# lmcinnes/pynndescent

Measured on AMD Instinct MI355X. Metric: index build: points indexed/sec (recall@10 vs brute force reported alongside), higher is better.
Workload: dtype f32

## Files before the change

include/pynnd_amd.h:

```cpp
#ifndef PYNND_AMD_H
#define PYNND_AMD_H

#include <stdint.h>

#ifdef __cplusplus
extern "C" {
#endif

#define NND_METRIC_SQEUCLIDEAN 0
#define NND_METRIC_ALT_COSINE 1
#define NND_METRIC_ALT_DOT 2
#define NND_METRIC_ALT_INNER_PRODUCT 3
#define NND_METRIC_CORRELATION 4
#define NND_METRIC_ALT_HELLINGER 5
enum { NND_METRIC_PROXY_INNER_PRODUCT = 6 };

#define NND_ABI_VERSION 6

typedef struct nnd_handle_s *nnd_handle_t;

typedef struct nnd_params {
    int64_t n;
    int32_t dim;
    int32_t metric;
    int32_t n_neighbors;
    int32_t n_trees;
    int32_t leaf_size;
    int32_t max_depth;
    int32_t max_candidates;
    int32_t n_iters;
    float delta;
    int64_t rng_state[3];
    int64_t tree_rng[3];
    int32_t device;
    int32_t join_blocks;
    int32_t flags;
    int32_t reserved[5];
} nnd_params;

#define NND_FLAG_NO_GRAPH 1
#define NND_FLAG_NO_PREP 2
#define NND_FLAG_TEST_SELECT_WAVE 4
#define NND_FLAG_TEST_SMALL_REGIONS 8
#define NND_FLAG_TEST_ROUTE_PLAIN 16
#define NND_FLAG_TEST_FOREST_BY_TREE 32
#define NND_FLAG_TEST_FAIL 64
#define NND_FLAG_TEST_VANISH 128
#define NND_FLAG_TEST_SAMPLE_ATOMIC 256
#define NND_FLAG_TEST_FOREST_FALLBACK_TOPS 512
#define NND_FLAG_TEST_FOREST_FALLBACK_SHARE 1024
#define NND_TEST_FALLBACK_AT(flags) ((((flags) & 512) ? 1 : 0) + (((flags) & 1024) ? 2 : 0))
#define NND_FLAG_TEST_SAMPLE_NOMEM 2048
#define NND_FLAG_TEST_SELECT_HALF 4096
#define NND_FLAG_TEST_GATHER_INLINE 8192
#define NND_FLAG_TEST_JOIN_UNSTAGED 16384

#define NND_FLAG_TEST_EXACT_F64 32768

typedef struct nnd_stats {
    int64_t n_iters_run;
    int64_t n_leaves;
    int64_t tree_levels;
    int64_t leaf_pairs;
    int64_t leaf_rows;
    int64_t join_pairs[64];
    int64_t join_rows[64];
    int64_t join_active[64];
    int64_t proposals[64];
    int64_t updates[64];
    float ms_prep, ms_forest, ms_leaf_init, ms_random_init, ms_descent, ms_finalize;
    float ms_sample[64], ms_join[64], ms_merge[64];
    int64_t join_mfma[64];
    int64_t leaf_mfma;
    int64_t n_cells;
    int64_t join_substeps[64];
} nnd_stats;

int32_t nnd_abi_version(void);
const char *nnd_last_global_error(void);
const char *nnd_last_error(nnd_handle_t h);

int32_t nnd_create(nnd_handle_t *out, const nnd_params *params);
int32_t nnd_destroy(nnd_handle_t h);
int32_t nnd_release_pending(void);

int32_t nnd_host_copy(void *dst, const void *src, int64_t bytes);
int32_t nnd_host_sqrt_f32(float *dst, const float *src, int64_t count);
void *nnd_host_alloc(int64_t bytes);
int32_t nnd_host_free(void *p);

int32_t nnd_set_data_host(nnd_handle_t h, const float *x);
int32_t nnd_set_data_device(nnd_handle_t h, const float *x_dev);
#define NND_DTYPE_FLOAT32 0
#define NND_DTYPE_FLOAT16 1
#define NND_DTYPE_BFLOAT16 2
#define NND_DTYPE_FLOAT64 3
int32_t nnd_set_data_device_typed(nnd_handle_t h, const void *x_dev, int32_t dtype);
int32_t nnd_device_rows_f32(int32_t device, void *hip_stream, const void *src_dev, int32_t dtype, int64_t n, int32_t dim,
                            int32_t normalize, float *dst_dev);
#define NND_CORRECT_COPY 0
#define NND_CORRECT_SQRT 1
#define NND_CORRECT_ALT_COSINE 2
#define NND_CORRECT_ALT_INNER_PRODUCT 3
#define NND_CORRECT_ALT_HELLINGER 4
int32_t nnd_device_correct(int32_t device, void *hip_stream, int32_t kind, const float *in_dev, void *out_dev, int64_t count);
int32_t nnd_device_update_rows(int32_t device, void *hip_stream, int32_t dim, const void *old_dev, int32_t old_dtype, int64_t n_old,
                               const void *fresh_dev, int32_t fresh_dtype, int64_t n_fresh, const void *upd_dev, int32_t upd_dtype,
                               int64_t n_upd, const int32_t *upd_rows_dev, const int32_t *upd_ids_dev, int64_t n_pairs, void *out_dev,
                               int32_t out_dtype);
int32_t nnd_device_update_graph(int32_t device, void *hip_stream, const int32_t *idx_dev, const float *dist_dev, int64_t n_old, int32_t k,
                                const int32_t *upd_ids_dev, int64_t n_upd, int64_t n_new, uint8_t *map_dev, int32_t *out_idx_dev,
                                float *out_dist_dev);
int32_t nnd_device_recall_hits(int32_t device, void *hip_stream, const int32_t *true_idx_dev, int64_t m, int32_t k, const int32_t *graph_idx_dev,
                               int64_t n, int32_t width, const int32_t *rows_dev, int64_t *hits_dev);
int32_t nnd_data_nonfinite(nnd_handle_t h, int32_t *out);
int32_t nnd_data_negative(nnd_handle_t h, int32_t *out);

int32_t nnd_make_forest(nnd_handle_t h);
int32_t nnd_leaf_array_shape(nnd_handle_t h, int64_t *n_leaves, int32_t *max_leaf_size);
int32_t nnd_get_leaf_array(nnd_handle_t h, int32_t *out_host);

int32_t nnd_reset_graph(nnd_handle_t h);
int32_t nnd_init_from_leaves(nnd_handle_t h);
int32_t nnd_init_from_leaf_array(nnd_handle_t h, const int32_t *leaf_array, int64_t n_leaves, int32_t max_leaf_size);
int32_t nnd_init_random(nnd_handle_t h);
int32_t nnd_init_from_graph(nnd_handle_t h, const int32_t *init_idx, const float *init_dist, int32_t width);
int32_t nnd_init_from_neighbor_graph(nnd_handle_t h, const int32_t *init_idx, const float *init_dist, int32_t width);
int32_t nnd_init_from_graph_device(nnd_handle_t h, const int32_t *init_idx_dev, const float *init_dist_dev, int32_t width);
int32_t nnd_init_from_neighbor_graph_device(nnd_handle_t h, const int32_t *init_idx_dev, const float *init_dist_dev, int32_t width);

int32_t nnd_descent_iter(nnd_handle_t h, int64_t *c_out);
int32_t nnd_descent(nnd_handle_t h);

int32_t nnd_finalize_host(nnd_handle_t h, int32_t *out_idx, float *out_dist);
int32_t nnd_finalize_device(nnd_handle_t h, int32_t *out_idx_dev, float *out_dist_dev);

int32_t nnd_build_device(nnd_handle_t h, int32_t *out_idx_dev, float *out_dist_dev);

int32_t nnd_build(const nnd_params *params, const float *x, const int32_t *init_idx, const float *init_dist,
                  int32_t init_width, int32_t *out_idx, float *out_dist, nnd_stats *stats, char *err,
// ... 167 lines not shown
```

pynndescent_amd/_capi.py:

```python
import ctypes as C
import os

import numpy as np

_HERE = os.path.dirname(os.path.abspath(__file__))
LIB_PATH = os.environ.get("PYNND_AMD_LIB", os.path.join(_HERE, "libpynnd_amd.so"))

NND_METRIC_SQEUCLIDEAN = 0
NND_METRIC_ALT_COSINE = 1
NND_METRIC_ALT_DOT = 2
NND_METRIC_ALT_INNER_PRODUCT = 3
NND_METRIC_CORRELATION = 4
NND_METRIC_ALT_HELLINGER = 5
NND_METRIC_PROXY_INNER_PRODUCT = 6
METRIC_CODES = {"euclidean": NND_METRIC_SQEUCLIDEAN, "l2": NND_METRIC_SQEUCLIDEAN, "sqeuclidean": NND_METRIC_SQEUCLIDEAN,
                "cosine": NND_METRIC_ALT_COSINE, "dot": NND_METRIC_ALT_DOT, "inner_product": NND_METRIC_ALT_INNER_PRODUCT,
                "correlation": NND_METRIC_CORRELATION, "hellinger": NND_METRIC_ALT_HELLINGER,
                "proxy_inner_product": NND_METRIC_PROXY_INNER_PRODUCT}
NND_DTYPE_FLOAT32, NND_DTYPE_FLOAT16, NND_DTYPE_BFLOAT16, NND_DTYPE_FLOAT64 = 0, 1, 2, 3
NND_CORRECT_COPY, NND_CORRECT_SQRT, NND_CORRECT_ALT_COSINE, NND_CORRECT_ALT_INNER_PRODUCT, NND_CORRECT_ALT_HELLINGER = 0, 1, 2, 3, 4
NND_FLAG_NO_GRAPH = 1
NND_FLAG_NO_PREP = 2
NND_FLAG_TEST_SELECT_WAVE = 4
NND_FLAG_TEST_SMALL_REGIONS = 8
NND_FLAG_TEST_ROUTE_PLAIN = 16
NND_FLAG_TEST_FOREST_BY_TREE = 32
NND_FLAG_TEST_FAIL = 64
NND_FLAG_TEST_VANISH = 128
NND_FLAG_TEST_FOREST_FALLBACK_TOPS = 512
NND_FLAG_TEST_FOREST_FALLBACK_SHARE = 1024
NND_FLAG_TEST_GATHER_INLINE = 8192
NND_FLAG_TEST_JOIN_UNSTAGED = 16384
NND_FLAG_TEST_SELECT_HALF = 4096
NND_FLAG_TEST_SAMPLE_NOMEM = 2048
NND_FLAG_TEST_EXACT_F64 = 32768
NND_FLAG_TEST_SAMPLE_ATOMIC = 256


class NNDParams(C.Structure):
    _fields_ = [
        ("n", C.c_int64),
        ("dim", C.c_int32),
        ("metric", C.c_int32),
        ("n_neighbors", C.c_int32),
        ("n_trees", C.c_int32),
        ("leaf_size", C.c_int32),
        ("max_depth", C.c_int32),
        ("max_candidates", C.c_int32),
        ("n_iters", C.c_int32),
        ("delta", C.c_float),
        ("rng_state", C.c_int64 * 3),
        ("tree_rng", C.c_int64 * 3),
        ("device", C.c_int32),
        ("join_blocks", C.c_int32),
        ("flags", C.c_int32),
        ("reserved", C.c_int32 * 5),
    ]


class NNDSearchGraphStats(C.Structure):
    _fields_ = [("forward_nnz", C.c_int64), ("reverse_nnz", C.c_int64), ("union_nnz", C.c_int64), ("final_nnz", C.c_int64),
                ("min_distance", C.c_float), ("max_degree_out", C.c_int32), ("ms_device", C.c_float), ("reserved", C.c_int32 * 3)]


class NNDStats(C.Structure):
    _fields_ = [
        ("n_iters_run", C.c_int64),
        ("n_leaves", C.c_int64),
        ("tree_levels", C.c_int64),
        ("leaf_pairs", C.c_int64),
        ("leaf_rows", C.c_int64),
        ("join_pairs", C.c_int64 * 64),
        ("join_rows", C.c_int64 * 64),
        ("join_active", C.c_int64 * 64),
        ("proposals", C.c_int64 * 64),
        ("updates", C.c_int64 * 64),
        ("ms_prep", C.c_float),
        ("ms_forest", C.c_float),
        ("ms_leaf_init", C.c_float),
        ("ms_random_init", C.c_float),
        ("ms_descent", C.c_float),
        ("ms_finalize", C.c_float),
        ("ms_sample", C.c_float * 64),
        ("ms_join", C.c_float * 64),
        ("ms_merge", C.c_float * 64),
        ("join_mfma", C.c_int64 * 64),
        ("leaf_mfma", C.c_int64),
        ("n_cells", C.c_int64),
        ("join_substeps", C.c_int64 * 64),
    ]

    def as_dict(self):
        it = int(self.n_iters_run)
        m = min(it, 64)
        out = {
            "n_iters_run": it, "n_leaves": int(self.n_leaves), "tree_levels": int(self.tree_levels),
            "leaf_pairs": int(self.leaf_pairs), "leaf_rows": int(self.leaf_rows), "leaf_mfma": int(self.leaf_mfma), "n_cells": int(self.n_cells),
        }
        for name in ("join_pairs", "join_rows", "join_active", "proposals", "updates", "join_mfma", "join_substeps"):
            out[name] = [int(v) for v in getattr(self, name)[:m]]
        for name in ("ms_prep", "ms_forest", "ms_leaf_init", "ms_random_init", "ms_descent", "ms_finalize"):
            out[name] = float(getattr(self, name))
        for name in ("ms_sample", "ms_join", "ms_merge"):
            out[name] = [float(v) for v in getattr(self, name)[:m]]
        return out


class NNDShardInfo(C.Structure):
    _fields_ = [
        ("n_total", C.c_int64), ("own_lo", C.c_int64), ("own_hi", C.c_int64),
        ("world", C.c_int32), ("rank", C.c_int32), ("local_trees", C.c_int32), ("iters", C.c_int32),
        ("c", C.c_int64 * 64),
        ("offer_records", C.c_int64 * 64),
        ("proposal_records", C.c_int64 * 64),
        ("deferred", C.c_int64 * 64),
        ("dropped_offers", C.c_int64),
        ("bytes_sent", C.c_int64),
        ("ms_total", C.c_float), ("ms_allgather", C.c_float), ("ms_klist_exchange", C.c_float),
# ... 780 lines not shown
```

pynndescent_amd/csrc/finalize.hip:

```cpp
#include "common.h"
#include "metric.h"
#include "state.h"

template <int FAM>
__device__ __forceinline__ void fin_acc(int metric, double a, double b, double &dot, double &nx, double &ny) {
    nnd_ref_acc<FAM, NND_HELLINGER_F32>(metric, a, b, dot, nx, ny);
}
template <int FAM>
__device__ __forceinline__ float fin_value(int metric, double dot, double nx, double ny) {
    const double dt = nnd_group_sum_f64<16>(dot);
    if (metric == 0) return (float)dt;
    return (float)nnd_ref_dist<FAM>(metric, dt, nnd_group_sum_f64<16>(nx), nnd_group_sum_f64<16>(ny));
}

template <int METRIC>
__global__ __launch_bounds__(256, METRIC == 0 ? 6 : 4) void k_finalize(const float *__restrict__ x, int d, int64_t lo, int64_t n, int k, int ks,
                                                  const uint32_t *__restrict__ knn_e, const int32_t *__restrict__ order,
                                                  int32_t *__restrict__ out_idx, float *__restrict__ out_dist) {
    const int lane = nnd_lane(), w = threadIdx.x >> 6;
    int64_t b = blockIdx.x;
    if ((gridDim.x & 7) == 0) b = (b & 7) * (gridDim.x >> 3) + (b >> 3);
    const int64_t g = lo + b * 4 + w;
    if (g >= n) return;
    const int64_t v = order ? (int64_t)order[g] : g;
    uint32_t e = lane < k ? knn_e[v * ks + lane] : NND_EMPTY_E;
    const float *xv = x + v * d;
    const int grp = lane >> 4, l16 = lane & 15;
    const bool vec = (d & 3) == 0;
    constexpr int metric = METRIC, FAM = METRIC < 2 ? NND_CODES_01 : NND_CODES_ANY;
    float mine = INFINITY;
    const int nsteps = (k + 3) >> 2;
    for (int s0 = 0; s0 < nsteps; s0 += 4) {
        const float *xu[4];
        bool on[4];
        double dot[4], nx[4], ny[4];
#pragma unroll
        for (int u = 0; u < 4; u++) {
            const int j = 4 * (s0 + u) + grp;
            const uint32_t ej = __shfl(e, j & 63, 64);
            on[u] = j < k && ej != NND_EMPTY_E;
            xu[u] = x + (int64_t)(on[u] ? (ej & NND_IDX_MASK) : 0) * d;
            dot[u] = nx[u] = ny[u] = 0.0;
        }
        double mua = 0.0, mub[4] = {0.0, 0.0, 0.0, 0.0};
        if (metric == 4) {
            mua = nnd_row_mean_f64<16>(xv, d, l16);
#pragma unroll
            for (int u = 0; u < 4; u++) mub[u] = nnd_row_mean_f64<16>(xu[u], d, l16);
        }
        if (vec) {
            for (int t = 4 * l16; t < d; t += 64) {
                const float4 a = *(const float4 *)(xv + t);
                float4 q[4];
#pragma unroll
                for (int u = 0; u < 4; u++) q[u] = *(const float4 *)(xu[u] + t);
#pragma unroll
                for (int u = 0; u < 4; u++) {
                    const double a0 = a.x, a1 = a.y, a2 = a.z, a3 = a.w;
                    const double b0 = q[u].x, b1 = q[u].y, b2 = q[u].z, b3 = q[u].w;
                    if (metric == 0) {
                        dot[u] += (a0 - b0) * (a0 - b0) + (a1 - b1) * (a1 - b1) + (a2 - b2) * (a2 - b2) + (a3 - b3) * (a3 - b3);
                    } else if (metric == 1) {
                        dot[u] += a0 * b0 + a1 * b1 + a2 * b2 + a3 * b3;
                        nx[u] += a0 * a0 + a1 * a1 + a2 * a2 + a3 * a3;
                        ny[u] += b0 * b0 + b1 * b1 + b2 * b2 + b3 * b3;
                    } else {
                        fin_acc<FAM>(metric, a0 - mua, b0 - mub[u], dot[u], nx[u], ny[u]);
                        fin_acc<FAM>(metric, a1 - mua, b1 - mub[u], dot[u], nx[u], ny[u]);
                        fin_acc<FAM>(metric, a2 - mua, b2 - mub[u], dot[u], nx[u], ny[u]);
                        fin_acc<FAM>(metric, a3 - mua, b3 - mub[u], dot[u], nx[u], ny[u]);
                    }
                }
            }
        } else {
            for (int t = l16; t < d; t += 16) {
                const double a0 = xv[t];
#pragma unroll
                for (int u = 0; u < 4; u++) {
                    fin_acc<FAM>(metric, a0 - mua, (double)xu[u][t] - mub[u], dot[u], nx[u], ny[u]);
                }
            }
        }
#pragma unroll
        for (int u = 0; u < 4; u++) {
            float val = fin_value<FAM>(metric, dot[u], nx[u], ny[u]);
            if (!on[u]) val = INFINITY;
            const float got = __shfl(val, 16 * (lane & 3), 64);
            if ((lane >> 2) == s0 + u) mine = got;
        }
    }
    const uint32_t myidx = e == NND_EMPTY_E ? NND_IDX_MASK : (e & NND_IDX_MASK);
    const uint64_t mykey = ((uint64_t)__float_as_uint(mine) << 32) | myidx;
    int r = 0;
    for (int j = 0; j < k; j++) {
        uint64_t kj = ((uint64_t)__float_as_uint(__shfl(mine, j, 64)) << 32) | __shfl(myidx, j, 64);
        r += (kj < mykey || (kj == mykey && j < lane)) ? 1 : 0;
    }
    if (lane < k) {
        out_idx[(v - lo) * k + r] = e == NND_EMPTY_E ? -1 : (int32_t)(e & NND_IDX_MASK);
        out_dist[(v - lo) * k + r] = mine;
    }
}

template <bool XM>
__global__ __launch_bounds__(256) void k_finalize_wide(const float *__restrict__ x, int d, int64_t lo, int64_t n, int k, int ks, int metric,
                                                       const uint32_t *__restrict__ knn_e, int32_t *__restrict__ out_idx,
                                                       float *__restrict__ out_dist) {
    __shared__ uint32_t sid[4][NND_WIDE_K];
    __shared__ float sdist[4][NND_WIDE_K];
    constexpr int FAM = XM ? NND_CODES_ANY : NND_CODES_01;
    const int lane = nnd_lane(), w = threadIdx.x >> 6, grp = lane >> 4, l16 = lane & 15;
    const int64_t v = lo + (int64_t)blockIdx.x * 4 + w;
    if (v >= n) return;
    for (int j = lane; j < k; j += 64) sid[w][j] = knn_e[v * ks + j];
    nnd_wave_lds_sync();
    const float *xv = x + v * d;
    for (int j0 = 0; j0 < k; j0 += 4) {
        const int j = j0 + grp;
        const uint32_t ej = j < k ? sid[w][j] : NND_EMPTY_E;
        const bool on = ej != NND_EMPTY_E;
        const float *xu = x + (int64_t)(on ? (ej & NND_IDX_MASK) : 0) * d;
        double dot = 0.0, nx = 0.0, ny = 0.0;
        const bool corr = XM && metric == 4;
        const double mua = corr ? nnd_row_mean_f64<16>(xv, d, l16) : 0.0, mub = corr ? nnd_row_mean_f64<16>(xu, d, l16) : 0.0;
        for (int t = l16; t < d; t += 16) fin_acc<FAM>(metric, (double)xv[t] - mua, (double)xu[t] - mub, dot, nx, ny);
        float val = fin_value<FAM>(metric, dot, nx, ny);
        if (!on) val = INFINITY;
        if (l16 == 0 && j < k) sdist[w][j] = val;
    }
    nnd_wave_lds_sync();
    for (int j = lane; j < k; j += 64) {
        const uint32_t e = sid[w][j];
        const uint32_t myidx = e == NND_EMPTY_E ? NND_IDX_MASK : (e & NND_IDX_MASK);
        const uint64_t mykey = ((uint64_t)__float_as_uint(sdist[w][j]) << 32) | myidx;
        int r = 0;
        for (int q = 0; q < k; q++) {
            const uint32_t eq = sid[w][q];
            const uint64_t kq = ((uint64_t)__float_as_uint(sdist[w][q]) << 32) | (eq == NND_EMPTY_E ? NND_IDX_MASK : (eq & NND_IDX_MASK));
            r += (kq < mykey || (kq == mykey && q < j)) ? 1 : 0;
        }
        out_idx[(v - lo) * k + r] = e == NND_EMPTY_E ? -1 : (int32_t)(e & NND_IDX_MASK);
        out_dist[(v - lo) * k + r] = sdist[w][j];
    }
}

int nnd_launch_finalize(nnd_ctx *ctx, int32_t *out_idx_dev, float *out_dist_dev) {
    unsigned grid = (unsigned)((ctx->own_hi - ctx->own_lo + 3) / 4);
    if (ctx->k > 64) {
        hipLaunchKernelGGL(ctx->p.metric >= 2 ? k_finalize_wide<true> : k_finalize_wide<false>, dim3(grid), dim3(256), 0, ctx->stream, ctx->x_orig, ctx->d, ctx->own_lo, ctx->own_hi, ctx->k, ctx->ks,
                           ctx->p.metric, ctx->knn_e, out_idx_dev, out_dist_dev);
        NND_HIP_CHECK(hipGetLastError());
        return 0;
    }
    grid = (grid + 7u) & ~7u;
    auto kern = k_finalize<0>;
    switch (ctx->p.metric) {
        case 1: kern = k_finalize<1>; break;
        case 2: kern = k_finalize<2>; break;
        case 3: kern = k_finalize<3>; break;
        case 4: kern = k_finalize<4>; break;
        case 5: kern = k_finalize<5>; break;
        case 6: kern = k_finalize<6>; break;
    }
    hipLaunchKernelGGL(kern, dim3(grid), dim3(256), 0, ctx->stream, ctx->x_orig, ctx->d, ctx->own_lo, ctx->own_hi,
                       ctx->k, ctx->ks, ctx->knn_e, nnd_vertex_order(ctx), out_idx_dev, out_dist_dev);
    NND_HIP_CHECK(hipGetLastError());
    return 0;
}

__global__ __launch_bounds__(64) void k_pairwise(const float *__restrict__ xp, int dp, const float *__restrict__ nrm,
                                                 int metric, const int32_t *__restrict__ rows_a, int na,
                                                 const int32_t *__restrict__ rows_b, int nb, float *__restrict__ out) {
    const int lane = nnd_lane(), r16 = lane & 15, g = lane >> 4;
    const int ta = blockIdx.y, tb = blockIdx.x;
    int ia = ta * 16 + r16, ib = tb * 16 + r16;
    int ida = ia < na ? rows_a[ia] : -1, idb = ib < nb ? rows_b[ib] : -1;
    f32x4 acc = {0.f, 0.f, 0.f, 0.f};
    for (int t = 0; t < (dp >> 4); t++) {
        int c = 4 * t + g;
        float4 a = ida >= 0 ? *(const float4 *)(xp + (int64_t)ida * dp + 4 * c) : make_float4(0, 0, 0, 0);
        float4 b = idb >= 0 ? *(const float4 *)(xp + (int64_t)idb * dp + 4 * c) : make_float4(0, 0, 0, 0);
        acc = __builtin_amdgcn_mfma_f32_16x16x4f32(a.x, b.x, acc, 0, 0, 0);
        acc = __builtin_amdgcn_mfma_f32_16x16x4f32(a.y, b.y, acc, 0, 0, 0);
        acc = __builtin_amdgcn_mfma_f32_16x16x4f32(a.z, b.z, acc, 0, 0, 0);
        acc = __builtin_amdgcn_mfma_f32_16x16x4f32(a.w, b.w, acc, 0, 0, 0);
    }
    int col = tb * 16 + r16;
    float nbv = idb >= 0 ? nrm[idb] : 0.0f;
#pragma unroll
    for (int r = 0; r < 4; r++) {
        int row = ta * 16 + 4 * g + r;
        int idr = row < na ? rows_a[row] : -1;
        if (row < na && col < nb) out[(int64_t)row * nb + col] = nnd_gram_to_dist<NND_CODES_ANY>(metric, acc[r], idr >= 0 ? nrm[idr] : 0.0f, nbv);
    }
}

int nnd_launch_pairwise(nnd_ctx *ctx, const int32_t *rows_a_dev, int na, const int32_t *rows_b_dev, int nb, float *out_dev) {
    dim3 grid((nb + 15) / 16, (na + 15) / 16);
    hipLaunchKernelGGL(k_pairwise, grid, dim3(64), 0, ctx->stream, ctx->xp, ctx->dp, ctx->nrm, ctx->p.metric, rows_a_dev, na,
                       rows_b_dev, nb, out_dev);
    NND_HIP_CHECK(hipGetLastError());
    return 0;
}
```

pynndescent_amd/csrc/merge.hip:

```cpp
#include "common.h"
#include "metric.h"
#include "merge.h"
#include "state.h"

__global__ __launch_bounds__(256) void k_merge(uint64_t *__restrict__ pbuf, uint8_t *__restrict__ pdirty, int pcap,
                                               int64_t lo, int64_t n, int k, int ks, uint32_t *__restrict__ knn_e,
                                               float *__restrict__ knn_d, float *__restrict__ th,
                                               long long *__restrict__ counters) {
    __shared__ int wacc[4];
    const int lane = nnd_lane(), w = threadIdx.x >> 6;
    const int64_t base = lo + ((int64_t)blockIdx.x * 4 + w) * 64;
    int acc = 0;
    unsigned long long m = 0;
    if (base < n) m = __ballot(base + lane < n && pdirty[base + lane < n ? base + lane : lo] != 0);
    struct pair_t {
        int64_t v[2];
        uint64_t key[2];
        uint32_t e[2];
        float d[2];
    };
    auto fetch = [&](pair_t &p) __attribute__((always_inline)) {
#pragma unroll
        for (int u = 0; u < 2; u++) {
            p.v[u] = -1;
// ... 74 lines not shown
    quad_t cur, nxt;
    cur.v = nxt.v = -1;
    bool have = m != 0;
    if (have) fetch(cur);
    while (have) {
        have = m != 0;
        if (have) fetch(nxt);
        const bool on = cur.v >= 0;
        const int64_t v = on ? cur.v : lo;
        const uint32_t e0 = on ? cur.e : NND_EMPTY_E;
        const float d0 = on ? cur.d : INFINITY;
        acc += nnd_merge_rows_q16<NB>(on, knn_e + v * ks, knn_d + v * ks, th + v, e0, d0, k, PCAP,
                                      [&](int c, uint32_t &id, float &dc) {
                                          const int b = c >> 4;
                                          const uint64_t kk = b == 0 ? cur.key[0] : (b == 1 ? cur.key[1] : (b == 2 ? cur.key[2] : cur.key[3]));
                                          id = nnd_key_idx(kk);
                                          dc = nnd_key_dist(kk);
                                          return kk != NND_EMPTY_KEY;
                                      });
        if (on) {
#pragma unroll
            for (int b = 0; b < NB; b++)
                if (cur.key[b] != NND_EMPTY_KEY) pbuf[v * PCAP + b * 16 + j] = NND_EMPTY_KEY;
            if (j == 0) pdirty[v] = 0;
        }
        cur = nxt;
    }
    if (lane == 0) wacc[w] = acc;
    __syncthreads();
    if (threadIdx.x == 0) {
        const long long a = (long long)wacc[0] + wacc[1] + wacc[2] + wacc[3];
        if (a) nnd_count(counters, CNT_ACCEPT, a);
    }
}

__global__ __launch_bounds__(256) void k_merge_wide(uint64_t *__restrict__ pbuf, uint8_t *__restrict__ pdirty, int pcap, int64_t lo, int64_t n,
                                                    int k, int ks, uint32_t *__restrict__ knn_e, float *__restrict__ knn_d,
                                                    float *__restrict__ th, long long *__restrict__ counters) {
    __shared__ uint64_t scr[4][NND_WIDE_SCRATCH_WORDS];
    __shared__ int wacc[4];
    const int lane = nnd_lane(), w = threadIdx.x >> 6;
    const int64_t base = lo + ((int64_t)blockIdx.x * 4 + w) * 64;
    int acc = 0;
    unsigned long long m = 0;
    if (base < n) m = __ballot(base + lane < n && pdirty[base + lane < n ? base + lane : lo] != 0);
    while (m) {
        const int64_t v = base + __builtin_ctzll(m);
        m &= m - 1;
        const uint64_t mykey = lane < pcap ? pbuf[v * pcap + lane] : NND_EMPTY_KEY;
        acc += nnd_merge_row_lds<1>(scr[w], knn_e + v * ks, knn_d + v * ks, th + v, k, pcap, [&](int c, uint32_t &id, float &dc) {
            id = nnd_key_idx(mykey);
            dc = nnd_key_dist(mykey);
            return mykey != NND_EMPTY_KEY;
        });
        if (lane < pcap && mykey != NND_EMPTY_KEY) pbuf[v * pcap + lane] = NND_EMPTY_KEY;
        if (lane == 0) pdirty[v] = 0;
        nnd_wave_lds_sync();
    }
    if (lane == 0) wacc[w] = acc;
    __syncthreads();
    if (threadIdx.x == 0) {
        const long long a = (long long)wacc[0] + wacc[1] + wacc[2] + wacc[3];
        if (a) nnd_count(counters, CNT_ACCEPT, a);
    }
}

int nnd_launch_merge(nnd_ctx *ctx) {
    if (ctx->pcap > 64) { ctx->set_error("k_merge expects at most 64 proposal slots per row"); return 1; }
    const dim3 grid((unsigned)((ctx->own_hi - ctx->own_lo + 255) / 256));
    if (ctx->k > NND_MAX_K)
        hipLaunchKernelGGL(k_merge_wide, grid, dim3(256), 0, ctx->stream, ctx->pbuf, ctx->pdirty, ctx->pcap, ctx->own_lo, ctx->own_hi, ctx->k,
                           ctx->ks, ctx->knn_e, ctx->knn_d, ctx->th, ctx->counters);
    else if (ctx->k <= 16 && ctx->pcap == 64)
        hipLaunchKernelGGL(k_merge_q, grid, dim3(256), 0, ctx->stream, ctx->pbuf, ctx->pdirty, ctx->own_lo, ctx->own_hi, ctx->k, ctx->ks,
                           ctx->knn_e, ctx->knn_d, ctx->th, ctx->counters);
    else
    hipLaunchKernelGGL(k_merge, grid, dim3(256), 0, ctx->stream, ctx->pbuf,
                       ctx->pdirty, ctx->pcap, ctx->own_lo, ctx->own_hi, ctx->k, ctx->ks, ctx->knn_e, ctx->knn_d, ctx->th, ctx->counters);
    NND_HIP_CHECK(hipGetLastError());
    if (ctx->n_ranks <= 1) ctx->pbuf_clean = true;
    return 0;
}

__global__ __launch_bounds__(256) void k_random_init(const float *__restrict__ xp, int dp, const float *__restrict__ nrm,
                                                     int metric, int64_t n, int64_t lo, int64_t hi, int k, int ks,
                                                     const uint32_t *__restrict__ knn_e, uint32_t seed,
                                                     uint64_t *__restrict__ pbuf, uint8_t *__restrict__ pdirty, int pcap) {
    const int lane = nnd_lane(), w = threadIdx.x >> 6;
    const int64_t v = lo + (int64_t)blockIdx.x * 4 + w;
    if (v >= hi) return;
    int filled = 0;
    for (int j0 = 0; j0 < k; j0 += 64) {
        const uint32_t e = j0 + lane < k ? knn_e[v * ks + j0 + lane] : NND_EMPTY_E;
        filled += __popcll(__ballot(e != NND_EMPTY_E));
    }
    int todo = k - filled;
    if (todo <= 0) return;
    if (todo > 64) todo = 64;
    uint32_t pick = (uint32_t)(nnd_hash3(seed, (uint32_t)v, (uint32_t)lane) % (uint64_t)n);
    bool mine = lane < todo;
    for (int j = 0; j < todo; j++) {
        uint32_t other = __shfl(pick, j, 64);
        if (j < lane && other == pick) mine = false;
    }
    for (int j = 0; j < todo; j++) {
        uint32_t id = __shfl(pick, j, 64);
        bool on = __shfl((int)mine, j, 64);
        if (!on) continue;
        float d = nnd_row_pair_dist(xp, dp, nrm, metric, v, (int64_t)id);
        if (lane == 0) pbuf[v * pcap + j] = nnd_make_key(d, id);
    }
    if (lane == 0) pdirty[v] = 1;
}

int nnd_launch_random_init(nnd_ctx *ctx) {
    for (int pass = 0; pass < (ctx->k + 63) / 64; pass++) {
        ctx->pbuf_clean = false;
        hipLaunchKernelGGL(k_random_init, dim3((unsigned)((ctx->own_hi - ctx->own_lo + 3) / 4)), dim3(256), 0, ctx->stream, ctx->xp,
                           ctx->dp, ctx->nrm, ctx->p.metric, ctx->n, ctx->own_lo, ctx->own_hi, ctx->k, ctx->ks, ctx->knn_e,
                           ctx->seed ^ 0x3C6EF372u ^ (uint32_t)(pass * 0x9E3779B9u), ctx->pbuf, ctx->pdirty, ctx->pcap);
        NND_HIP_CHECK(hipGetLastError());
        if (nnd_launch_merge(ctx)) return 1;
    }
    return 0;
}

__global__ __launch_bounds__(256) void k_graph_init(const float *__restrict__ xp, int dp, const float *__restrict__ nrm,
                                                    int metric, int64_t n, int64_t lo, int64_t hi, const int32_t *__restrict__ gidx,
                                                    const float *__restrict__ gdist, int width, int col0, int wchunk,
                                                    uint64_t *__restrict__ pbuf, uint8_t *__restrict__ pdirty, int pcap) {
    const int lane = nnd_lane(), w = threadIdx.x >> 6;
    const int64_t v = lo + (int64_t)blockIdx.x * 4 + w;
    if (v >= hi) return;
    gidx += -lo * width;
    if (gdist) gdist += -lo * width;
    int32_t id = lane < wchunk ? gidx[v * width + col0 + lane] : -1;
    bool mine = id >= 0 && (int64_t)id < n;
    for (int j = 0; j < wchunk; j++) {
        int32_t other = __shfl(id, j, 64);
        if (j < lane && other == id) mine = false;
    }
    for (int j = 0; j < wchunk; j++) {
        int32_t q = __shfl(id, j, 64);
        bool on = __shfl((int)mine, j, 64);
        if (!on) continue;
        float d = gdist ? nnd_clamp_dist(gdist[v * width + col0 + j]) : nnd_row_pair_dist(xp, dp, nrm, metric, v, (int64_t)q);
        if (lane == 0) pbuf[v * pcap + j] = nnd_make_key(d, (uint32_t)q);
    }
    if (lane == 0) pdirty[v] = 1;
}

int nnd_launch_init_from_graph(nnd_ctx *ctx, const int32_t *idx_dev, const float *dist_dev, int width) {
    if (ctx->pcap < 64) { ctx->set_error("init graphs need 64 proposal slots per row"); return 1; }
    const int64_t rows = ctx->own_hi - ctx->own_lo;
    if (rows <= 0) return 0;
    for (int col0 = 0; col0 < width; col0 += 64) {
        const int wchunk = width - col0 < 64 ? width - col0 : 64;
        ctx->pbuf_clean = false;
        hipLaunchKernelGGL(k_graph_init, dim3((unsigned)((rows + 3) / 4)), dim3(256), 0, ctx->stream, ctx->xp, ctx->dp,
                           ctx->nrm, ctx->p.metric, ctx->n, ctx->own_lo, ctx->own_hi, idx_dev, dist_dev, width, col0, wchunk, ctx->pbuf, ctx->pdirty,
                           ctx->pcap);
        NND_HIP_CHECK(hipGetLastError());
        if (nnd_launch_merge(ctx)) return 1;
    }
    return 0;
}

__global__ void k_clear_new_flags(uint32_t *__restrict__ knn_e, int64_t lo, int64_t hi, int ks) {
    int64_t t = lo * ks + (int64_t)blockIdx.x * blockDim.x + threadIdx.x;
    if (t >= hi * ks) return;
    const uint32_t e = knn_e[t];
    if (e != NND_EMPTY_E) knn_e[t] = e & NND_IDX_MASK;
}
int nnd_launch_clear_new_flags(nnd_ctx *ctx) {
    const int64_t total = (ctx->own_hi - ctx->own_lo) * ctx->ks;
    if (total <= 0) return 0;
    hipLaunchKernelGGL(k_clear_new_flags, dim3((unsigned)((total + 255) / 256)), dim3(256), 0, ctx->stream, ctx->knn_e,
                       ctx->own_lo, ctx->own_hi, ctx->ks);
    NND_HIP_CHECK(hipGetLastError());
    return 0;
}


__global__ void k_import_proposals(const uint64_t *__restrict__ keys, const int32_t *__restrict__ targets, int64_t count,
                                   uint64_t *__restrict__ pbuf, uint8_t *__restrict__ pdirty, int pcap, uint32_t slot_seed,
                                   const uint32_t *__restrict__ knn_e, const float *__restrict__ th, int ks) {
    const int64_t i = (int64_t)blockIdx.x * blockDim.x + threadIdx.x;
    if (i >= count) return;
    const uint64_t key = keys[i];
    const int64_t t = targets[i];
    if (t < 0) return;
    const uint32_t src = nnd_key_idx(key);
    if (!(nnd_key_dist(key) < th[t])) return;
    const u32x4 *row = (const u32x4 *)(knn_e + t * ks);
    bool present = false;
    for (int c = 0; c < (ks >> 2); c++) {
        const u32x4 wv = row[c] & NND_IDX_MASK;
        present |= (wv.x == src) | (wv.y == src) | (wv.z == src) | (wv.w == src);
    }
    if (present) return;
    const uint32_t s = nnd_hash2(slot_seed, src) & (uint32_t)(pcap - 1);
    atomicMin((unsigned long long *)&pbuf[t * pcap + s], (unsigned long long)key);
    pdirty[t] = 1;
// ... 260 lines not shown
```

pynndescent_amd/csrc/prep.hip:

```cpp
#include "common.h"
#include "metric.h"
#include "state.h"

#define NND_MEAN_ROWS 65536
__global__ void k_colsum_partial(const float *__restrict__ x, int64_t row0, int64_t r_lo, int64_t r_hi, int64_t stride, int d,
                                 int rows_per_block, double *__restrict__ partial) {
    __shared__ float wmax[4];
    int64_t r0 = r_lo + (int64_t)blockIdx.x * rows_per_block;
    int64_t r1 = r0 + rows_per_block < r_hi ? r0 + rows_per_block : r_hi;
    float mx = 0.0f;
    for (int j = threadIdx.x; j < d; j += blockDim.x) {
        double s = 0.0;
        for (int64_t r = r0; r < r1; r++) {
            const float v = x[(r * stride - row0) * d + j];
            s += (double)v;
            mx = fmaxf(mx, fabsf(v));
        }
        partial[(int64_t)blockIdx.x * (d + 1) + j] = s;
    }
#pragma unroll
    for (int o = 32; o > 0; o >>= 1) mx = fmaxf(mx, __shfl_xor(mx, o, 64));
    if (nnd_lane() == 0) wmax[threadIdx.x >> 6] = mx;
    __syncthreads();
    if (threadIdx.x == 0) {
// ... 200 lines not shown
        hipLaunchKernelGGL(k_colsum_final, dim3(dp + 1), dim3(256), 0, ctx->stream, partial, nblocks, d, dp, n_s, ctx->mean);
    } else {
        NND_HIP_CHECK(hipMemsetAsync(ctx->mean, 0, sizeof(float) * (dp + 4), ctx->stream));
    }
    hipLaunchKernelGGL(k_screen_scale, dim3(1), dim3(64), 0, ctx->stream, ctx->mean, d, dp, ctx->p.metric);
    NND_HIP_CHECK(hipGetLastError());
    return 0;
}
int nnd_prep_partial_blocks(int64_t members) { return (int)((members + 127) / 128); }
double *nnd_prep_partial_buffer(nnd_ctx *ctx, size_t doubles) {
    if (!ctx->mem.grow(&ctx->colsum_partial, &ctx->colsum_cap, doubles, doubles)) ctx->set_error("allocation of the column-sum scratch failed");
    return ctx->colsum_partial;
}
int nnd_prep_rows(nnd_ctx *ctx, const float *x_all, int64_t row_lo, int64_t row_hi, bool first) {
    const int d = ctx->d, dp = ctx->dp;
    const int64_t rows = row_hi - row_lo;
    long long *flag = ctx->counters_sum + CNT_PREP_FLAG;
    if (first) NND_HIP_CHECK(hipMemsetAsync(flag, 0, sizeof(long long), ctx->stream));
    if (rows <= 0) return 0;
    if ((d & 3) == 0 && ((uintptr_t)x_all & 15) == 0) {
        int lpr = 1;
        while (lpr < (dp >> 2) && lpr < 64) lpr <<= 1;
        const int64_t rows_per_wg = 4 * (64 / lpr);
        hipLaunchKernelGGL(k_prep_rows_v4, dim3((unsigned)((rows + rows_per_wg - 1) / rows_per_wg)), dim3(256), 0, ctx->stream, x_all, row_lo, row_hi, d,
                           dp, ctx->p.metric, lpr, ctx->mean, ctx->xp, ctx->nrm, ctx->xh, ctx->nr2, flag);
    } else {
        hipLaunchKernelGGL(k_prep_rows, dim3((unsigned)((rows + 3) / 4)), dim3(256), 0, ctx->stream, x_all, row_lo, row_hi, d, dp,
                           ctx->p.metric, ctx->mean, ctx->xp, ctx->nrm, ctx->xh, ctx->nr2, flag);
    }
    NND_HIP_CHECK(hipGetLastError());
    return 0;
}

int nnd_launch_prep(nnd_ctx *ctx) {
    const int64_t n = ctx->n;
    int64_t n_s, stride;
    nnd_prep_mean_geometry(n, &n_s, &stride);
    int nblocks = 0;
    double *partial = nullptr;
    if (nnd_prep_column_pass(ctx->p.metric)) {
        partial = nnd_prep_partial_buffer(ctx, (size_t)nnd_prep_partial_blocks(n_s) * (ctx->d + 1));
        if (!partial) return 1;
        nblocks = nnd_prep_mean_partial(ctx, ctx->x_orig, 0, 0, n_s, stride, partial);
    }
    if (nnd_prep_mean_finish(ctx, partial, nblocks, n_s)) return 1;
    if (nnd_prep_rows(ctx, ctx->x_orig, 0, n, true)) return 1;
    long long *flag = ctx->counters_sum + CNT_PREP_FLAG;
    NND_HIP_CHECK(hipMemcpyAsync(&ctx->h_pin->data_flags, flag, sizeof(long long), hipMemcpyDeviceToHost, ctx->stream));
    return 0;
}

__global__ void k_reset_graph(uint32_t *__restrict__ e, float *__restrict__ dd, int64_t total, float *__restrict__ th,
                              int64_t n) {
    int64_t i = (int64_t)blockIdx.x * blockDim.x + threadIdx.x;
    if (i < total) {
        e[i] = NND_EMPTY_E;
        dd[i] = INFINITY;
    }
    if (i < n) th[i] = INFINITY;
}

int nnd_launch_reset_graph(nnd_ctx *ctx) {
    ctx->all_new = true;
    ctx->last_updates = -1;
    int64_t total = ctx->n * ctx->ks;
    hipLaunchKernelGGL(k_reset_graph, dim3((unsigned)((total + 255) / 256)), dim3(256), 0, ctx->stream, ctx->knn_e,
                       ctx->knn_d, total, ctx->th, ctx->n);
    if (!ctx->pbuf_clean) {
        NND_HIP_CHECK(hipMemsetAsync(ctx->pbuf + (size_t)ctx->slim_row0() * ctx->pcap, 0xFF, sizeof(uint64_t) * (size_t)ctx->slim_rows() * ctx->pcap, ctx->stream));
        if (ctx->pbuf_r) NND_HIP_CHECK(hipMemsetAsync(ctx->pbuf_r, 0xFF, sizeof(uint64_t) * (size_t)ctx->n * ctx->pcap_r, ctx->stream));
    }
    if (!ctx->rbuf_clean)
        NND_HIP_CHECK(hipMemsetAsync(ctx->rbuf + (size_t)ctx->slim_row0() * 2 * ctx->rcap, 0xFF, sizeof(uint32_t) * (size_t)ctx->slim_rows() * 2 * ctx->rcap, ctx->stream));
    ctx->pbuf_clean = ctx->rbuf_clean = true;
    NND_HIP_CHECK(hipGetLastError());
    ctx->iter = 0;
    return 0;
}

int nnd_zero_counters(nnd_ctx *ctx) {
    NND_HIP_CHECK(hipMemsetAsync(ctx->counters, 0, sizeof(long long) * CNT_COUNT * NND_CNT_STRIPES, ctx->stream));
    return 0;
}
__global__ __launch_bounds__(256) void k_counters_reduce(const long long *__restrict__ counters, long long *__restrict__ out) {
    __shared__ long long red[256];
    for (int c = 0; c < CNT_COUNT; c++) {
        long long s = 0;
        for (int i = threadIdx.x; i < NND_CNT_STRIPES; i += 256) s += counters[(size_t)i * CNT_COUNT + c];
        red[threadIdx.x] = s;
        __syncthreads();
        for (int o = 128; o > 0; o >>= 1) {
            if (threadIdx.x < o) red[threadIdx.x] += red[threadIdx.x + o];
            __syncthreads();
        }
        if (threadIdx.x == 0) out[c] = red[0];
        __syncthreads();
    }
}
int nnd_read_counters(nnd_ctx *ctx) {
    hipLaunchKernelGGL(k_counters_reduce, dim3(1), dim3(256), 0, ctx->stream, ctx->counters, ctx->counters_sum);
    NND_HIP_CHECK(hipGetLastError());
    NND_HIP_CHECK(hipMemcpyAsync(ctx->h_pin->counters, ctx->counters_sum, sizeof(long long) * CNT_COUNT, hipMemcpyDeviceToHost, ctx->stream));
    NND_HIP_CHECK(nnd_sync_spin(ctx));
    for (int c = 0; c < CNT_COUNT; c++) ctx->h_counters[c] = ctx->h_pin->counters[c];
    return 0;
}
```

Baseline: 51.91 million.

## Add 16-lane finalize kernel, ballot-skip full rows in random init, wave-reduce counters

```diff
diff --git a/include/pynnd_amd.h b/include/pynnd_amd.h
--- a/include/pynnd_amd.h
+++ b/include/pynnd_amd.h
@@ -56,6 +56,7 @@
 #define NND_FLAG_TEST_JOIN_UNSTAGED 16384
 
 #define NND_FLAG_TEST_EXACT_F64 32768
+#define NND_FLAG_TEST_RANDOM_INIT_ROWWISE 65536
 
 typedef struct nnd_stats {
     int64_t n_iters_run;
diff --git a/pynndescent_amd/_capi.py b/pynndescent_amd/_capi.py
--- a/pynndescent_amd/_capi.py
+++ b/pynndescent_amd/_capi.py
@@ -34,6 +34,7 @@
 NND_FLAG_TEST_SELECT_HALF = 4096
 NND_FLAG_TEST_SAMPLE_NOMEM = 2048
 NND_FLAG_TEST_EXACT_F64 = 32768
+NND_FLAG_TEST_RANDOM_INIT_ROWWISE = 65536
 NND_FLAG_TEST_SAMPLE_ATOMIC = 256
 
 
diff --git a/pynndescent_amd/csrc/finalize.hip b/pynndescent_amd/csrc/finalize.hip
--- a/pynndescent_amd/csrc/finalize.hip
+++ b/pynndescent_amd/csrc/finalize.hip
@@ -1,6 +1,31 @@
 #include "common.h"
+#include "merge.h"
 #include "metric.h"
 #include "state.h"
+
+__device__ __forceinline__ double fin_sub(double a, double b) {
+#pragma clang fp contract(off)
+    return a - b;
+}
+__device__ __forceinline__ double fin_add(double a, double b) {
+#pragma clang fp contract(off)
+    return a + b;
+}
+__device__ __forceinline__ double fin_chunk(double a0, double a1, double a2, double a3, double b0, double b1, double b2, double b3) {
+#pragma clang fp contract(off)
+    double s = a1 * b1;
+    s = __builtin_fma(a0, b0, s);
+    s = __builtin_fma(a2, b2, s);
+    return __builtin_fma(a3, b3, s);
+}
+__device__ __forceinline__ double fin_chunk_sq(const float4 a, const float4 b) {
+    const double d0 = fin_sub((double)a.x, (double)b.x), d1 = fin_sub((double)a.y, (double)b.y);
+    const double d2 = fin_sub((double)a.z, (double)b.z), d3 = fin_sub((double)a.w, (double)b.w);
+    return fin_chunk(d0, d1, d2, d3, d0, d1, d2, d3);
+}
+__device__ __forceinline__ double fin_chunk_dot(const float4 a, const float4 b) {
+    return fin_chunk((double)a.x, (double)a.y, (double)a.z, (double)a.w, (double)b.x, (double)b.y, (double)b.z, (double)b.w);
+}
 
 template <int FAM>
 __device__ __forceinline__ void fin_acc(int metric, double a, double b, double &dot, double &nx, double &ny) {
@@ -56,15 +81,15 @@
                 for (int u = 0; u < 4; u++) q[u] = *(const float4 *)(xu[u] + t);
 #pragma unroll
                 for (int u = 0; u < 4; u++) {
-                    const double a0 = a.x, a1 = a.y, a2 = a.z, a3 = a.w;
-                    const double b0 = q[u].x, b1 = q[u].y, b2 = q[u].z, b3 = q[u].w;
                     if (metric == 0) {
-                        dot[u] += (a0 - b0) * (a0 - b0) + (a1 - b1) * (a1 - b1) + (a2 - b2) * (a2 - b2) + (a3 - b3) * (a3 - b3);
+                        dot[u] = fin_add(dot[u], fin_chunk_sq(a, q[u]));
                     } else if (metric == 1) {
-                        dot[u] += a0 * b0 + a1 * b1 + a2 * b2 + a3 * b3;
-                        nx[u] += a0 * a0 + a1 * a1 + a2 * a2 + a3 * a3;
-                        ny[u] += b0 * b0 + b1 * b1 + b2 * b2 + b3 * b3;
+                        dot[u] = fin_add(dot[u], fin_chunk_dot(a, q[u]));
+                        nx[u] = fin_add(nx[u], fin_chunk_dot(a, a));
+                        ny[u] = fin_add(ny[u], fin_chunk_dot(q[u], q[u]));
                     } else {
+                        const double a0 = a.x, a1 = a.y, a2 = a.z, a3 = a.w;
+                        const double b0 = q[u].x, b1 = q[u].y, b2 = q[u].z, b3 = q[u].w;
                         fin_acc<FAM>(metric, a0 - mua, b0 - mub[u], dot[u], nx[u], ny[u]);
                         fin_acc<FAM>(metric, a1 - mua, b1 - mub[u], dot[u], nx[u], ny[u]);
                         fin_acc<FAM>(metric, a2 - mua, b2 - mub[u], dot[u], nx[u], ny[u]);
@@ -97,6 +122,107 @@
         r += (kj < mykey || (kj == mykey && j < lane)) ? 1 : 0;
     }
     if (lane < k) {
+        out_idx[(v - lo) * k + r] = e == NND_EMPTY_E ? -1 : (int32_t)(e & NND_IDX_MASK);
+        out_dist[(v - lo) * k + r] = mine;
+    }
+}
+
+template <int CTRL>
+__device__ __forceinline__ double fin_dpp_f64(double v) {
+    const uint64_t b = (uint64_t)__double_as_longlong(v);
+    const uint32_t lo = (uint32_t)__builtin_amdgcn_update_dpp(0, (int)(uint32_t)b, CTRL, 0xF, 0xF, true);
+    const uint32_t hi = (uint32_t)__builtin_amdgcn_update_dpp(0, (int)(uint32_t)(b >> 32), CTRL, 0xF, 0xF, true);
+    return __longlong_as_double((long long)(((uint64_t)hi << 32) | lo));
+}
+__device__ __forceinline__ double fin_row_sum_f64(double v) {
+    v = fin_add(v, fin_dpp_f64<NND_DPP_ROW_ROR(8)>(v));
+    v = fin_add(v, fin_dpp_f64<NND_DPP_ROW_HALF_MIRROR>(v));
+    v = fin_add(v, fin_dpp_f64<NND_DPP_QUAD_XOR2>(v));
+    return fin_add(v, fin_dpp_f64<NND_DPP_QUAD_XOR1>(v));
+}
+__device__ __forceinline__ double fin_row_sum4_f64(const double (&v)[4], int p16) {
+    const bool lo8 = (p16 & 8) == 0, lo4 = (p16 & 4) == 0;
+    const double a = fin_add(lo8 ? v[0] : v[2], fin_dpp_f64<NND_DPP_ROW_ROR(8)>(lo8 ? v[2] : v[0]));
+    const double b = fin_add(lo8 ? v[1] : v[3], fin_dpp_f64<NND_DPP_ROW_ROR(8)>(lo8 ? v[3] : v[1]));
+    double s = fin_add(lo4 ? a : b, fin_dpp_f64<NND_DPP_ROW_HALF_MIRROR>(lo4 ? b : a));
+    s = fin_add(s, fin_dpp_f64<NND_DPP_QUAD_XOR2>(s));
+    return fin_add(s, fin_dpp_f64<NND_DPP_QUAD_XOR1>(s));
+}
+template <int T>
+__device__ __forceinline__ int fin_row_rank(uint32_t klo, uint32_t khi, int p16) {
+    if constexpr (T == 0) return 0;
+    else {
+        const uint32_t olo = (uint32_t)__builtin_amdgcn_update_dpp(0, (int)klo, NND_DPP_ROW_ROR(T), 0xF, 0xF, true);
+        const uint32_t ohi = (uint32_t)__builtin_amdgcn_update_dpp(0, (int)khi, NND_DPP_ROW_ROR(T), 0xF, 0xF, true);
+        const uint64_t other = ((uint64_t)ohi << 32) | olo, mine = ((uint64_t)khi << 32) | klo;
+        return (((other < mine) | ((other == mine) & (p16 >= T))) ? 1 : 0) + fin_row_rank<T - 1>(klo, khi, p16);
+    }
+}
+
+template <int METRIC>
+__global__ __launch_bounds__(256, METRIC == 0 ? 6 : 4) void k_finalize16(const float *__restrict__ x, int d, int64_t lo, int64_t n, int k, int ks,
+                                                    const uint32_t *__restrict__ knn_e, const int32_t *__restrict__ order,
+                                                    int32_t *__restrict__ out_idx, float *__restrict__ out_dist) {
+    static_assert(METRIC == 0 || METRIC == 1, "the other codes go through k_finalize");
+    const int lane = nnd_lane(), w = threadIdx.x >> 6, grp = lane >> 4, p16 = lane & 15;
+    const int c16 = (p16 & 4) ? (p16 ^ 3) : p16;
+    int64_t b = blockIdx.x;
+    if ((gridDim.x & 7) == 0) b = (b & 7) * (gridDim.x >> 3) + (b >> 3);
+    const int64_t g0 = lo + (b * 4 + w) * 4;
+    if (g0 >= n) return;
+    const bool row_on = g0 + grp < n;
+    const int64_t g = row_on ? g0 + grp : n - 1;
+    const int64_t v = order ? (int64_t)order[g] : g;
+    const uint32_t *er = knn_e + v * ks;
+    const int j16 = 4 * (p16 & 3) + (p16 >> 2);
+    const uint32_t e = j16 < k ? er[j16] : NND_EMPTY_E;
+    u32x4 eb[4];
+#pragma unroll
+    for (int bt = 0; bt < 4; bt++) eb[bt] = *(const u32x4 *)(er + 4 * bt);
+    const uint32_t row_bytes = (uint32_t)d * 4u;
+    const char *xc = (const char *)(x + 4 * c16);
+    const float *xv = (const float *)(xc + (uint64_t)v * row_bytes);
+    float mine = INFINITY;
+#pragma unroll
+    for (int bt = 0; bt < 4; bt++) {
+        if (4 * bt >= k) break;
+        const float *xu[4];
+        double dot[4], ny[4], nx = 0.0;
+#pragma unroll
+        for (int u = 0; u < 4; u++) {
+            const uint32_t ej = eb[bt][u];
+            const bool on = 4 * bt + u < k && ej != NND_EMPTY_E;
+            xu[u] = (const float *)(xc + (uint64_t)(on ? (ej & NND_IDX_MASK) : 0u) * row_bytes);
+            dot[u] = ny[u] = 0.0;
+        }
+        for (int t = 4 * c16; t < d; t += 64) {
+            const int o = t - 4 * c16;
+            const float4 a = *(const float4 *)(xv + o);
+            float4 q[4];
+#pragma unroll
+            for (int u = 0; u < 4; u++) q[u] = *(const float4 *)(xu[u] + o);
+            if (METRIC == 1) nx = fin_add(nx, fin_chunk_dot(a, a));
+#pragma unroll
+            for (int u = 0; u < 4; u++) {
+                if (METRIC == 0) {
+                    dot[u] = fin_add(dot[u], fin_chunk_sq(a, q[u]));
+                } else {
+                    dot[u] = fin_add(dot[u], fin_chunk_dot(a, q[u]));
+                    ny[u] = fin_add(ny[u], fin_chunk_dot(q[u], q[u]));
+                }
+            }
+        }
+        const double dt = fin_row_sum4_f64(dot, p16);
+        float val;
+        if (METRIC == 0) val = (float)dt;
+        else val = (float)nnd_ref_dist<NND_CODES_01>(1, dt, fin_row_sum_f64(nx), fin_row_sum4_f64(ny, p16));
+        if ((p16 & 3) == bt) mine = val;
+    }
+    if (e == NND_EMPTY_E) mine = INFINITY;
+    const uint32_t myidx = e == NND_EMPTY_E ? NND_IDX_MASK : (e & NND_IDX_MASK);
+    const uint32_t klo = j16 < k ? myidx : 0xFFFFFFFFu, khi = j16 < k ? __float_as_uint(mine) : 0xFFFFFFFFu;
+    const int r = fin_row_rank<15>(klo, khi, p16);
+    if (row_on && j16 < k) {
         out_idx[(v - lo) * k + r] = e == NND_EMPTY_E ? -1 : (int32_t)(e & NND_IDX_MASK);
         out_dist[(v - lo) * k + r] = mine;
     }
@@ -152,6 +278,13 @@
         NND_HIP_CHECK(hipGetLastError());
         return 0;
     }
+    if (ctx->k <= 16 && ctx->p.metric <= 1 && (ctx->d & 3) == 0) {
+        grid = ((unsigned)((ctx->own_hi - ctx->own_lo + 15) / 16) + 7u) & ~7u;
+        hipLaunchKernelGGL(ctx->p.metric == 0 ? k_finalize16<0> : k_finalize16<1>, dim3(grid), dim3(256), 0, ctx->stream, ctx->x_orig, ctx->d,
+                           ctx->own_lo, ctx->own_hi, ctx->k, ctx->ks, ctx->knn_e, nnd_vertex_order(ctx), out_idx_dev, out_dist_dev);
+        NND_HIP_CHECK(hipGetLastError());
+        return 0;
+    }
     grid = (grid + 7u) & ~7u;
     auto kern = k_finalize<0>;
     switch (ctx->p.metric) {
diff --git a/pynndescent_amd/csrc/merge.hip b/pynndescent_amd/csrc/merge.hip
--- a/pynndescent_amd/csrc/merge.hip
+++ b/pynndescent_amd/csrc/merge.hip
@@ -180,13 +180,10 @@
     return 0;
 }
 
-__global__ __launch_bounds__(256) void k_random_init(const float *__restrict__ xp, int dp, const float *__restrict__ nrm,
-                                                     int metric, int64_t n, int64_t lo, int64_t hi, int k, int ks,
-                                                     const uint32_t *__restrict__ knn_e, uint32_t seed,
-                                                     uint64_t *__restrict__ pbuf, uint8_t *__restrict__ pdirty, int pcap) {
-    const int lane = nnd_lane(), w = threadIdx.x >> 6;
-    const int64_t v = lo + (int64_t)blockIdx.x * 4 + w;
-    if (v >= hi) return;
+__device__ __forceinline__ void random_init_row(const float *__restrict__ xp, int dp, const float *__restrict__ nrm, int metric, int64_t n,
+                                                int64_t v, int k, int ks, const uint32_t *__restrict__ knn_e, uint32_t seed,
+                                                uint64_t *__restrict__ pbuf, uint8_t *__restrict__ pdirty, int pcap) {
+    const int lane = nnd_lane();
     int filled = 0;
     for (int j0 = 0; j0 < k; j0 += 64) {
         const uint32_t e = j0 + lane < k ? knn_e[v * ks + j0 + lane] : NND_EMPTY_E;
@@ -210,13 +207,47 @@
     }
     if (lane == 0) pdirty[v] = 1;
 }
+__global__ __launch_bounds__(256) void k_random_init(const float *__restrict__ xp, int dp, const float *__restrict__ nrm,
+                                                     int metric, int64_t n, int64_t lo, int64_t hi, int k, int ks,
+                                                     const uint32_t *__restrict__ knn_e, uint32_t seed,
+                                                     uint64_t *__restrict__ pbuf, uint8_t *__restrict__ pdirty, int pcap) {
+    const int lane = nnd_lane(), w = threadIdx.x >> 6;
+    const int64_t base = lo + ((int64_t)blockIdx.x * 4 + w) * 64;
+    if (base >= hi) return;
+    int filled = k;
+    if (base + lane < hi) {
+        filled = 0;
+        const u32x4 *row = (const u32x4 *)(knn_e + (base + lane) * ks);
+        for (int c = 0; 4 * c < k; c++) {
+            const u32x4 e = row[c];
+#pragma unroll
+            for (int q = 0; q < 4; q++) filled += (4 * c + q < k && e[q] != NND_EMPTY_E) ? 1 : 0;
+        }
+    }
+    unsigned long long m = __ballot(filled < k);
+    while (m) {
+        const int64_t v = base + __builtin_ctzll(m);
+        m &= m - 1;
+        random_init_row(xp, dp, nrm, metric, n, v, k, ks, knn_e, seed, pbuf, pdirty, pcap);
+    }
+}
+__global__ __launch_bounds__(256) void k_random_init_rowwise(const float *__restrict__ xp, int dp, const float *__restrict__ nrm,
+                                                             int metric, int64_t n, int64_t lo, int64_t hi, int k, int ks,
+                                                             const uint32_t *__restrict__ knn_e, uint32_t seed,
+                                                             uint64_t *__restrict__ pbuf, uint8_t *__restrict__ pdirty, int pcap) {
+    const int64_t v = lo + (int64_t)blockIdx.x * 4 + (threadIdx.x >> 6);
+    if (v >= hi) return;
+    random_init_row(xp, dp, nrm, metric, n, v, k, ks, knn_e, seed, pbuf, pdirty, pcap);
+}
 
 int nnd_launch_random_init(nnd_ctx *ctx) {
+    const bool rowwise = (ctx->p.flags & NND_FLAG_TEST_RANDOM_INIT_ROWWISE) != 0;
+    const int64_t rows = ctx->own_hi - ctx->own_lo;
     for (int pass = 0; pass < (ctx->k + 63) / 64; pass++) {
         ctx->pbuf_clean = false;
-        hipLaunchKernelGGL(k_random_init, dim3((unsigned)((ctx->own_hi - ctx->own_lo + 3) / 4)), dim3(256), 0, ctx->stream, ctx->xp,
-                           ctx->dp, ctx->nrm, ctx->p.metric, ctx->n, ctx->own_lo, ctx->own_hi, ctx->k, ctx->ks, ctx->knn_e,
-                           ctx->seed ^ 0x3C6EF372u ^ (uint32_t)(pass * 0x9E3779B9u), ctx->pbuf, ctx->pdirty, ctx->pcap);
+        hipLaunchKernelGGL(rowwise ? k_random_init_rowwise : k_random_init, dim3((unsigned)(rowwise ? (rows + 3) / 4 : (rows + 255) / 256)),
+                           dim3(256), 0, ctx->stream, ctx->xp, ctx->dp, ctx->nrm, ctx->p.metric, ctx->n, ctx->own_lo, ctx->own_hi, ctx->k,
+                           ctx->ks, ctx->knn_e, ctx->seed ^ 0x3C6EF372u ^ (uint32_t)(pass * 0x9E3779B9u), ctx->pbuf, ctx->pdirty, ctx->pcap);
         NND_HIP_CHECK(hipGetLastError());
         if (nnd_launch_merge(ctx)) return 1;
     }
diff --git a/pynndescent_amd/csrc/prep.hip b/pynndescent_amd/csrc/prep.hip
--- a/pynndescent_amd/csrc/prep.hip
+++ b/pynndescent_amd/csrc/prep.hip
@@ -306,23 +306,16 @@
     NND_HIP_CHECK(hipMemsetAsync(ctx->counters, 0, sizeof(long long) * CNT_COUNT * NND_CNT_STRIPES, ctx->stream));
     return 0;
 }
-__global__ __launch_bounds__(256) void k_counters_reduce(const long long *__restrict__ counters, long long *__restrict__ out) {
-    __shared__ long long red[256];
-    for (int c = 0; c < CNT_COUNT; c++) {
-        long long s = 0;
-        for (int i = threadIdx.x; i < NND_CNT_STRIPES; i += 256) s += counters[(size_t)i * CNT_COUNT + c];
-        red[threadIdx.x] = s;
-        __syncthreads();
-        for (int o = 128; o > 0; o >>= 1) {
-            if (threadIdx.x < o) red[threadIdx.x] += red[threadIdx.x + o];
-            __syncthreads();
-        }
-        if (threadIdx.x == 0) out[c] = red[0];
-        __syncthreads();
-    }
+__global__ __launch_bounds__(64 * CNT_COUNT) void k_counters_reduce(const long long *__restrict__ counters, long long *__restrict__ out) {
+    const int lane = nnd_lane(), c = threadIdx.x >> 6;
+    long long s = 0;
+    for (int i = lane; i < NND_CNT_STRIPES; i += 64) s += counters[(size_t)i * CNT_COUNT + c];
+#pragma unroll
+    for (int o = 32; o > 0; o >>= 1) s += __shfl_xor(s, o, 64);
+    if (lane == 0) out[c] = s;
 }
 int nnd_read_counters(nnd_ctx *ctx) {
-    hipLaunchKernelGGL(k_counters_reduce, dim3(1), dim3(256), 0, ctx->stream, ctx->counters, ctx->counters_sum);
+    hipLaunchKernelGGL(k_counters_reduce, dim3(1), dim3(64 * CNT_COUNT), 0, ctx->stream, ctx->counters, ctx->counters_sum);
     NND_HIP_CHECK(hipGetLastError());
     NND_HIP_CHECK(hipMemcpyAsync(ctx->h_pin->counters, ctx->counters_sum, sizeof(long long) * CNT_COUNT, hipMemcpyDeviceToHost, ctx->stream));
     NND_HIP_CHECK(nnd_sync_spin(ctx));
```

Result: faster. 53.22 million, median of 6 (+2.5%).
